# quziyan/NPairLoss

Hardware: NVIDIA H100
Metric: N-pair fwd+bwd samples/sec at B=8192,D=512 (higher is better)
Workload: dtype f32 (3-pass fp16-split wgmma, f32 accumulate)

## Files before the change

### npairloss_b200/csrc/gemm_wgmma.cuh

```cuda
#pragma once
#include <cuda.h>
#include <cuda_runtime.h>
#include <cfloat>
#include <stdint.h>

#include "kernels.cuh"
#include "ptx.cuh"
#include "thresholds.cuh"

namespace npair {

enum { EPI_SIM = 0, EPI_OUT = 1, EPI_SIM_SYM = 2, EPI_SIM_STATS = 3, EPI_SIM_SYM_STATS = 4, EPI_SIM_STORE = 5 };
__host__ __device__ constexpr bool epi_sym(int e) { return e == EPI_SIM_SYM || e == EPI_SIM_SYM_STATS; }
__host__ __device__ constexpr bool epi_stores_s(int e) { return e == EPI_SIM || e == EPI_SIM_SYM || e == EPI_SIM_STORE; }
__host__ __device__ constexpr bool epi_stats(int e) { return e != EPI_OUT && e != EPI_SIM_STORE; }

struct GemmParams {
  int M, Nn;
  int num_kblocks;
  int tiles_m, tiles_n;
  const int2* tile_list;
  int num_tiles_list;
  int splits, kb_per_split;
  float* part;
  float* S;
  long long ldS;
  const float* dev_scale;
  const float* lab_rows;
  const float* lab_cols;
  int self_offset;
  uint32_t* st_minw;
  uint32_t* st_maxw;
  uint32_t* st_maxb;
  uint32_t* st_maxall;
  int* cnt_same;
  int fuse_thr;
  RowArrays ra;
  MiningParams mp;
  BlockScalars* bs;
  float* out;
  long long ldo;
  float alpha, beta;
  int a_row0;
};

template <int NSPLIT, int BK_, int EPI>
struct GemmCfg {
  static constexpr int BM = 128, BN = 256;
  static constexpr int BK = BK_;
  static constexpr int ROW_BYTES = BK * 2;
  static constexpr uint32_t LAYOUT = (ROW_BYTES == 128) ? 1u : 2u;
  static constexpr uint32_t SBO = 8 * ROW_BYTES;
  static constexpr int A_PIECE = BM * ROW_BYTES;
  static constexpr int B_PIECE = BN * ROW_BYTES;
  static constexpr int STAGE_BYTES = NSPLIT * (A_PIECE + B_PIECE);
  static constexpr int NPASS = (NSPLIT == 1) ? 1 : (NSPLIT == 2 ? 3 : 6);
  static constexpr int ACC_STAGE_BYTES = (EPI != EPI_OUT) ? 2 * 64 * 64 * 4 : 0;
  static constexpr int STORE_STAGE_BYTES = (EPI != EPI_OUT) ? 8 * 4096 : 0;
  static constexpr int SMEM_AUX = 2048;
  static constexpr int SMEM_MAX = 227 * 1024;
  static constexpr int STAGES_FIT = (SMEM_MAX - SMEM_AUX - 1024 - ACC_STAGE_BYTES - STORE_STAGE_BYTES) / STAGE_BYTES;
  static constexpr int STAGES = STAGES_FIT > 6 ? 6 : STAGES_FIT;
  static constexpr int SMEM_BYTES = STAGES * STAGE_BYTES + ACC_STAGE_BYTES + STORE_STAGE_BYTES + SMEM_AUX + 1024 ;
  static constexpr int THREADS = 384;
  static_assert(STAGES >= 2 && 16 * STAGES <= 192, "operand ring");
};

__device__ __forceinline__ void pass_pieces(int nsplit, int p, int& sa, int& sb) {
  if (nsplit == 1) { sa = 0; sb = 0; return; }
  if (nsplit == 2) { sa = (p == 2) ? 1 : 0; sb = (p == 1) ? 1 : 0; return; }
  const int A[6] = {0, 0, 1, 1, 0, 2};
  const int B[6] = {0, 1, 0, 1, 2, 0};
  sa = A[p]; sb = B[p];
}

__device__ __forceinline__ void stats32(const float (&v)[32], const float* __restrict__ lab, float lab_i, bool fast, int idx0,
                                        int limit, int self_idx, float& minw, float& maxw, float& maxb, int& cnt) {
  if (fast) {
    float mnw[4] = {FLT_MAX, FLT_MAX, FLT_MAX, FLT_MAX}, mxw[4] = {-FLT_MAX, -FLT_MAX, -FLT_MAX, -FLT_MAX};
    float mxb[4] = {-FLT_MAX, -FLT_MAX, -FLT_MAX, -FLT_MAX};
    int cn[4] = {0, 0, 0, 0};
#pragma unroll
    for (int q = 0; q < 8; ++q) {
      const float4 l4 = *reinterpret_cast<const float4*>(lab + 4 * q);
      const float ll[4] = {l4.x, l4.y, l4.z, l4.w};
#pragma unroll
      for (int e = 0; e < 4; ++e) {
        const float x = v[4 * q + e];
        if (ll[e] == lab_i) { mnw[e] = fminf(mnw[e], x); mxw[e] = fmaxf(mxw[e], x); ++cn[e]; }
        else mxb[e] = fmaxf(mxb[e], x);
      }
    }
    minw = fminf(minw, fminf(fminf(mnw[0], mnw[1]), fminf(mnw[2], mnw[3])));
    maxw = fmaxf(maxw, fmaxf(fmaxf(mxw[0], mxw[1]), fmaxf(mxw[2], mxw[3])));
    maxb = fmaxf(maxb, fmaxf(fmaxf(mxb[0], mxb[1]), fmaxf(mxb[2], mxb[3])));
    cnt += (cn[0] + cn[1]) + (cn[2] + cn[3]);
  } else {
#pragma unroll
    for (int c = 0; c < 32; ++c) {
      const int idx = idx0 + c;
      const bool valid = (idx < limit) && (idx != self_idx);
      const bool same = (lab[c] == lab_i);
      if (valid && same) { minw = fminf(minw, v[c]); maxw = fmaxf(maxw, v[c]); ++cnt; }
      if (valid && !same) maxb = fmaxf(maxb, v[c]);
    }
  }
}

__device__ __forceinline__ float max32(const float (&v)[32]) {
  float m[8];
#pragma unroll
  for (int e = 0; e < 8; ++e) m[e] = fmaxf(fmaxf(v[e], v[8 + e]), fmaxf(v[16 + e], v[24 + e]));
  return fmaxf(fmaxf(fmaxf(m[0], m[1]), fmaxf(m[2], m[3])), fmaxf(fmaxf(m[4], m[5]), fmaxf(m[6], m[7])));
}

template <int NSPLIT, bool BF16, int EPI, int BK_>
__global__ void __launch_bounds__(384, 1)
split_gemm_kernel(const __grid_constant__ CUtensorMap tmapA, const __grid_constant__ CUtensorMap tmapB,
                  const __grid_constant__ CUtensorMap tmapS, const GemmParams p) {
  using Cfg = GemmCfg<NSPLIT, BK_, EPI>;
  const int worker = static_cast<int>(blockIdx.x), num_workers = static_cast<int>(gridDim.x);
  constexpr int BM = Cfg::BM, BN = Cfg::BN, BK = Cfg::BK, STAGES = Cfg::STAGES;
  constexpr bool SYM = epi_sym(EPI), STORE = epi_stores_s(EPI), STATS = epi_stats(EPI);
  extern __shared__ uint8_t smem_raw[];
  uint8_t* smem = smem_raw + ((1024u - (ptx::smem_u32(smem_raw) & 1023u)) & 1023u);
  uint8_t* acc_stage = smem + STAGES * Cfg::STAGE_BYTES;
  uint8_t* store_stage = acc_stage + Cfg::ACC_STAGE_BYTES;
  uint8_t* aux = store_stage + Cfg::STORE_STAGE_BYTES;
  uint64_t* full_bar = reinterpret_cast<uint64_t*>(aux);
  uint64_t* empty_bar = full_bar + STAGES;
  float* s_lab = reinterpret_cast<float*>(aux + 256);
  float* s_labr = reinterpret_cast<float*>(aux + 256 + 1024);
  float2* s_rng = reinterpret_cast<float2*>(aux + 256 + 1024 + 512);

  const int warp = threadIdx.x >> 5, lane = threadIdx.x & 31;
  const int num_tiles = p.tile_list ? p.num_tiles_list : p.tiles_m * p.tiles_n * p.splits;
  const float inv_scale = p.dev_scale ? *p.dev_scale : 1.f;
  const float out_scale = (EPI != EPI_OUT) ? inv_scale * inv_scale : 1.f;
  const float alpha = p.alpha * inv_scale;

  if (warp == 0 && lane == 0) {
    ptx::prefetch_tmap(&tmapA);
    ptx::prefetch_tmap(&tmapB);
    if (STORE) ptx::prefetch_tmap(&tmapS);
  }
  if (warp == 1 && lane == 0) {
    for (int s = 0; s < STAGES; ++s) { ptx::mbar_init(&full_bar[s], 1); ptx::mbar_init(&empty_bar[s], 8); }
    ptx::fence_mbar_init();
  }
  __syncthreads();

  if (warp == 0) {
    if (lane == 0) {
      int stage = 0; uint32_t phase = 0;
      for (int tile = worker; tile < num_tiles; tile += num_workers) {
        const int mn = tile / p.splits, split = tile - mn * p.splits;
        int m_blk = mn / p.tiles_n, n_blk = mn % p.tiles_n;
        if (p.tile_list) { const int2 tl = p.tile_list[tile]; m_blk = tl.x; n_blk = tl.y; }
        const int kb0 = split * p.kb_per_split, kb1 = min(p.num_kblocks, kb0 + p.kb_per_split);
        for (int kb = kb0; kb < kb1; ++kb) {
          ptx::mbar_wait(&empty_bar[stage], phase ^ 1);
          uint8_t* st = smem + stage * Cfg::STAGE_BYTES;
          ptx::mbar_arrive_expect_tx(&full_bar[stage], Cfg::STAGE_BYTES);
#pragma unroll
          for (int s = 0; s < NSPLIT; ++s) {
            ptx::tma_load_3d(st + s * Cfg::A_PIECE, &tmapA, &full_bar[stage], kb * BK, m_blk * BM + (EPI == EPI_SIM_STORE ? p.a_row0 : 0), s);
            ptx::tma_load_3d(st + NSPLIT * Cfg::A_PIECE + s * Cfg::B_PIECE, &tmapB, &full_bar[stage], kb * BK, n_blk * BN, s);
          }
          if (++stage == STAGES) { stage = 0; phase ^= 1; }
        }
      }
    }
  } else if (warp >= 4) {
    const int cw = warp - 4;
    const int g = cw >> 2, wi = warp & 3;
    const int ew = 2 * g + (wi & 1);
    const int half = wi >> 1;
    const int et = threadIdx.x - 128;
    uint8_t* const accs = acc_stage + g * (64 * 256);
    uint8_t* const stg = store_stage + cw * 4096;
    int stage = 0; uint32_t phase = 0;
    for (int tile = worker; tile < num_tiles; tile += num_workers) {
      const int mn = tile / p.splits, split = tile - mn * p.splits;
      int m_blk = mn / p.tiles_n, n_blk = mn % p.tiles_n;
      if (p.tile_list) { const int2 tl = p.tile_list[tile]; m_blk = tl.x; n_blk = tl.y; }
      const int kb0 = split * p.kb_per_split, kb1 = min(p.num_kblocks, kb0 + p.kb_per_split);
      const int row = m_blk * BM + ew * 32 + lane;
      const int col_base = n_blk * BN;
      float lab_i = 0.f;
      if (STATS) {
        asm volatile("bar.sync 1, 256;" ::: "memory");
        s_lab[et] = (col_base + et < p.Nn) ? p.lab_cols[col_base + et] : 0.f;
        if (row < p.M) lab_i = p.lab_rows[row];
        if (SYM && half == 0) s_labr[ew * 32 + lane] = lab_i;
        asm volatile("bar.sync 1, 256;" ::: "memory");
        {
          const float lc = s_lab[cw * 32 + lane];
          float mn = lc, mx = lc;
#pragma unroll
          for (int o = 16; o > 0; o >>= 1) { mn = fminf(mn, __shfl_xor_sync(0xffffffffu, mn, o)); mx = fmaxf(mx, __shfl_xor_sync(0xffffffffu, mx, o)); }
          if (lane == 0) s_rng[cw] = make_float2(mn, mx);
          if (SYM && cw < 4) {
            const float lr = s_labr[cw * 32 + lane];
            float rn = lr, rx = lr;
#pragma unroll
            for (int o = 16; o > 0; o >>= 1) { rn = fminf(rn, __shfl_xor_sync(0xffffffffu, rn, o)); rx = fmaxf(rx, __shfl_xor_sync(0xffffffffu, rx, o)); }
            if (lane == 0) s_rng[8 + cw] = make_float2(rn, rx);
          }
        }
        asm volatile("bar.sync 1, 256;" ::: "memory");
      }

      float acc[128];
#pragma unroll
      for (int i = 0; i < 128; ++i) acc[i] = 0.f;
      for (int kb = kb0; kb < kb1; ++kb) {
        ptx::mbar_wait(&full_bar[stage], phase);
        const uint32_t a0 = ptx::smem_u32(smem + stage * Cfg::STAGE_BYTES) + g * 64 * Cfg::ROW_BYTES;
        const uint32_t b0 = ptx::smem_u32(smem + stage * Cfg::STAGE_BYTES) + NSPLIT * Cfg::A_PIECE;
        ptx::wgmma_fence();
#pragma unroll
        for (int ps = 0; ps < Cfg::NPASS; ++ps) {
          int sa, sb;
          pass_pieces(NSPLIT, ps, sa, sb);
#pragma unroll
          for (int k4 = 0; k4 < BK / 16; ++k4) {
            const uint64_t ad = ptx::make_kmajor_desc(a0 + sa * Cfg::A_PIECE + k4 * 32, Cfg::SBO, Cfg::LAYOUT);
            const uint64_t bd = ptx::make_kmajor_desc(b0 + sb * Cfg::B_PIECE + k4 * 32, Cfg::SBO, Cfg::LAYOUT);
            ptx::wgmma_m64n256k16_ss<BF16>(acc, ad, bd, 1u);
          }
        }
        ptx::wgmma_commit();
        ptx::wgmma_wait<0>();
        ptx::fence_regs(acc);
        __syncwarp();
        if (lane == 0) ptx::mbar_arrive(&empty_bar[stage]);
        if (++stage == STAGES) { stage = 0; phase ^= 1; }
      }

      if (EPI == EPI_OUT) {
        float* obase = p.splits > 1 ? p.part + static_cast<long long>(split) * p.M * p.ldo : p.out;
        const float beta = p.splits > 1 ? 0.f : p.beta;
        const int rbase = m_blk * BM + g * 64 + wi * 16 + (lane >> 2);
#pragma unroll
        for (int j = 0; j < 32; ++j) {
          const int col = col_base + 8 * j + 2 * (lane & 3);
#pragma unroll
          for (int h = 0; h < 2; ++h) {
            const int r = rbase + 8 * h;
            if (r >= p.M || col >= p.Nn) continue;
            float* dst = obase + static_cast<long long>(r) * p.ldo + col;
            float o0 = alpha * acc[4 * j + 2 * h], o1 = alpha * acc[4 * j + 2 * h + 1];
            if (col + 1 < p.Nn && (p.ldo & 1) == 0) {
              if (beta != 0.f) { const float2 old = *reinterpret_cast<const float2*>(dst); o0 += beta * old.x; o1 += beta * old.y; }
              *reinterpret_cast<float2*>(dst) = make_float2(o0, o1);
            } else {
              dst[0] = (beta != 0.f) ? o0 + beta * dst[0] : o0;
              if (col + 1 < p.Nn) dst[1] = (beta != 0.f) ? o1 + beta * dst[1] : o1;
            }
          }
        }
        continue;
      }

      float minw = FLT_MAX, maxw = -FLT_MAX, maxb = -FLT_MAX, maxall = -FLT_MAX;
      int cnt = 0;
      const int self_col = row + p.self_offset;
      const int srow = (wi & 1) * 32 + lane;
#pragma unroll
      for (int cp = 0; cp < 4; ++cp) {
        asm volatile("bar.sync %0, 128;" ::"r"(2 + g) : "memory");
        {
          const int c = lane & 3;
#pragma unroll
          for (int j = 0; j < 8; ++j) {
            const int q = 2 * j + (c >> 1);
#pragma unroll
            for (int h = 0; h < 2; ++h) {
              const int r = wi * 16 + (lane >> 2) + 8 * h;
              *reinterpret_cast<float2*>(accs + r * 256 + ((q ^ (r & 7)) << 4) + (c & 1) * 8) =
                  make_float2(acc[4 * (8 * cp + j) + 2 * h], acc[4 * (8 * cp + j) + 2 * h + 1]);
            }
          }
        }
        asm volatile("bar.sync %0, 128;" ::"r"(2 + g) : "memory");
        const int ch = 2 * cp + half;
        const int col0 = col_base + ch * 32;
        const int cb = col0 >> 7;
        if ((SYM && cb < m_blk) || col0 >= p.Nn) continue;
        float v[32];
        if (STATS) {
#pragma unroll
          for (int q = 0; q < 8; ++q) {
            const float4 t4 = *reinterpret_cast<const float4*>(accs + srow * 256 + (((half * 8 + q) ^ (srow & 7)) << 4));
            v[4 * q] = t4.x * out_scale; v[4 * q + 1] = t4.y * out_scale; v[4 * q + 2] = t4.z * out_scale; v[4 * q + 3] = t4.w * out_scale;
          }
        }
        if (STORE) {
          const int cq = lane & 7;
#pragma unroll
          for (int i = 0; i < 8; ++i) {
            const int rr = 4 * i + (lane >> 3);
            const int grow = m_blk * BM + ew * 32 + rr;
            const int sr = (wi & 1) * 32 + rr;
            float4 o = *reinterpret_cast<const float4*>(accs + sr * 256 + (((half * 8 + cq) ^ (sr & 7)) << 4));
            o.x *= out_scale; o.y *= out_scale; o.z *= out_scale; o.w *= out_scale;
            if (grow < p.M) *reinterpret_cast<float4*>(p.S + static_cast<long long>(grow) * p.ldS + col0 + 4 * cq) = o;
          }
        }
        if (STATS) {
          const float2 rg = s_rng[ch];
          if (__all_sync(0xffffffffu, row >= p.M || lab_i < rg.x || lab_i > rg.y) && col0 + 32 <= p.Nn) {
            if (row < p.M) maxb = fmaxf(maxb, max32(v));
          } else if (row < p.M)
            stats32(v, s_lab + ch * 32, lab_i, col0 + 32 <= p.Nn && (self_col < col0 || self_col >= col0 + 32), col0, p.Nn, self_col,
                    minw, maxw, maxb, cnt);
        }
        if (SYM && cb > m_blk && m_blk * BM + ew * 32 < p.M) {
          if (STORE && lane == 0) ptx::tma_store_wait_read<0>();
          __syncwarp();
#pragma unroll
          for (int c = 0; c < 32; ++c)
            *reinterpret_cast<float*>(stg + c * 128 + ((((lane >> 2) ^ (c & 7))) << 4) + ((lane & 3) << 2)) = v[c];
          if (STORE) ptx::fence_proxy_async_smem();
          __syncwarp();
          if (STORE && lane == 0) { ptx::tma_store_2d(&tmapS, stg, m_blk * BM + ew * 32, col0); ptx::tma_store_commit(); }
          const int gc = col0 + lane;
          float vt[32];
#pragma unroll
          for (int q = 0; q < 8; ++q) {
            const float4 t4 = *reinterpret_cast<const float4*>(stg + lane * 128 + ((q ^ (lane & 7)) << 4));
            vt[4 * q] = t4.x; vt[4 * q + 1] = t4.y; vt[4 * q + 2] = t4.z; vt[4 * q + 3] = t4.w;
          }
          float t_minw = FLT_MAX, t_maxw = -FLT_MAX, t_maxb = -FLT_MAX;
          int t_cnt = 0;
          const int r0 = m_blk * BM + ew * 32;
          const float lab_c = s_lab[ch * 32 + lane];
          const float2 rr = s_rng[8 + ew];
          const bool plain = __all_sync(0xffffffffu, gc >= p.Nn || lab_c < rr.x || lab_c > rr.y) && r0 + 32 <= p.M;
          if (gc < p.Nn) {
            if (plain) t_maxb = max32(vt);
            else stats32(vt, s_labr + ew * 32, lab_c, r0 + 32 <= p.M, r0, p.M, -1, t_minw, t_maxw, t_maxb, t_cnt);
            if (t_cnt) {
              atomicMin(&p.st_minw[gc], f2ord(t_minw));
              atomicMax(&p.st_maxw[gc], f2ord(t_maxw));
              atomicAdd(&p.cnt_same[gc], t_cnt);
            }
            atomicMax(&p.st_maxb[gc], f2ord(t_maxb));
            atomicMax(&p.st_maxall[gc], f2ord(fmaxf(t_maxw, t_maxb)));
          }
        }
      }
      if (STATS && row < p.M) {
        maxall = fmaxf(maxw, maxb);
        if (cnt) {
          atomicMin(&p.st_minw[row], f2ord(minw));
          atomicMax(&p.st_maxw[row], f2ord(maxw));
          atomicAdd(&p.cnt_same[row], cnt);
        }
        atomicMax(&p.st_maxb[row], f2ord(maxb));
        atomicMax(&p.st_maxall[row], f2ord(maxall));
      }
    }
  }
  if (STORE && warp >= 4 && lane == 0) ptx::tma_store_wait<0>();
  __syncthreads();
  if (STATS && p.fuse_thr) {
    volatile int& s_last_cta = *reinterpret_cast<volatile int*>(aux + 192);
    __threadfence();
    __syncthreads();
    if (threadIdx.x == 0) s_last_cta = (atomicAdd(&p.bs->ticket2, 1u) == gridDim.x - 1) ? 1 : 0;
    __syncthreads();
    if (s_last_cta) {
      __threadfence();
      thresholds_one_block(p.ra, p.M, p.Nn, p.mp, p.bs, smem);
      if (threadIdx.x == 0) p.bs->ticket2 = 0;
    }
  }
}

}
```

### npairloss_b200/csrc/grad_fused.cuh

```cuda
#pragma once
#include <cuda.h>
#include <cuda_bf16.h>
#include <cuda_fp16.h>
#include <cuda_runtime.h>
#include <stdint.h>

#include "gemm_wgmma.cuh"
#include "ptx.cuh"

namespace npair {

#define NPAIR_LOG2E_F 1.4426950408889634f

struct FusedGradParams {
  int Q, N, D;
  int num_kblocks;
  int tiles_m, tiles_n;
  int splits, kb_per_split;
  int chunk_kb;
  float* part;
  const float* S;
  const float* rowrec;
  const float* colrec;
  int self_offset;
  float inv_world, log2_world;
  float sgn_p, sgn_n;
  float* out; long long ldo;
  float alpha, beta;
  const float* dev_scale;
  int m_blk0;
};

template <int NSPLIT>
struct FusedCfg {
  static constexpr int BM = 128, BN = 256, BK = 32;
  static constexpr int B_PIECE = BN * 64;
  static constexpr int S_TILE = BM * 128;
  static constexpr int CREC = BK * 32;
  static constexpr int STAGE_BYTES = NSPLIT * B_PIECE + S_TILE + CREC;
  static constexpr int NPASS = (NSPLIT == 1) ? 1 : (NSPLIT == 2 ? 3 : 6);
  static constexpr int STAGES_FIT = (227 * 1024 - 2048) / STAGE_BYTES;
  static constexpr int STAGES = STAGES_FIT > 6 ? 6 : STAGES_FIT;
  static constexpr int SMEM_BYTES = STAGES * STAGE_BYTES + 1024  + 1024 ;
  static constexpr int THREADS = 384;
};

template <int NSPLIT, bool BF16>
__device__ __forceinline__ void split_pair(float a, float b, uint32_t (&out)[3]) {
  if (NSPLIT == 1) {
    out[0] = static_cast<uint32_t>(__bfloat16_as_ushort(__float2bfloat16_rn(a))) | (static_cast<uint32_t>(__bfloat16_as_ushort(__float2bfloat16_rn(b))) << 16);
  } else if (NSPLIT == 2) {
    const __half2 h = __floats2half2_rn(a, b);
    const float2 hf = __half22float2(h);
    const __half2 l = __floats2half2_rn(a - hf.x, b - hf.y);
    out[0] = *reinterpret_cast<const uint32_t*>(&h);
    out[1] = *reinterpret_cast<const uint32_t*>(&l);
  } else {
    const __nv_bfloat162 h = __floats2bfloat162_rn(a, b);
    const float2 hf = __bfloat1622float2(h);
    const float r1a = a - hf.x, r1b = b - hf.y;
    const __nv_bfloat162 m = __floats2bfloat162_rn(r1a, r1b);
    const float2 mf = __bfloat1622float2(m);
    const __nv_bfloat162 l = __floats2bfloat162_rn(r1a - mf.x, r1b - mf.y);
    out[0] = *reinterpret_cast<const uint32_t*>(&h);
    out[1] = *reinterpret_cast<const uint32_t*>(&m);
    out[2] = *reinterpret_cast<const uint32_t*>(&l);
  }
}

__device__ __forceinline__ void red_add_v2(float* dst, float a, float b) {
  asm volatile("red.global.add.v2.f32 [%0], {%1, %2};" ::"l"(dst), "f"(a), "f"(b) : "memory");
}
__device__ __forceinline__ void red_add_f32(float* dst, float a) {
  asm volatile("red.global.add.f32 [%0], %1;" ::"l"(dst), "f"(a) : "memory");
}

__device__ __forceinline__ void bulk_copy_g2s(void* smem_dst, const void* gsrc, uint32_t bytes, uint64_t* bar) {
  asm volatile("cp.async.bulk.shared::cluster.global.mbarrier::complete_tx::bytes [%0], [%1], %2, [%3];"
               ::"r"(ptx::smem_u32(smem_dst)), "l"(reinterpret_cast<uint64_t>(gsrc)), "r"(bytes), "r"(ptx::smem_u32(bar))
               : "memory");
}

__device__ __forceinline__ int chunk_end(int c0, int kb0, int kb1, int ch, int key) {
  if (ch <= 0) return kb1;
  if (c0 == kb0) { const int first = max(1, (((key & 7) + 1) * ch) >> 3); return min(kb1, kb0 + first); }
  return min(kb1, c0 + ch);
}

struct RowRec { float m2r, tn, m2, lab, tp, cA; int self_col; };

__device__ __forceinline__ float pair_weight(float s, const float4* __restrict__ rec, const RowRec& r, int m, const FusedGradParams& p) {
  float g;
  const float4 ca = rec[0];
  if (ca.w != r.lab) {
    const float key = s * p.sgn_n;
    float e1, e2;
    asm("ex2.approx.ftz.f32 %0, %1;" : "=f"(e1) : "f"(key <= r.tn ? fmaf(s, NPAIR_LOG2E_F, -r.m2r) : -INFINITY));
    asm("ex2.approx.ftz.f32 %0, %1;" : "=f"(e2) : "f"(key <= ca.y ? fmaf(s, NPAIR_LOG2E_F, -ca.x) : -INFINITY));
    g = e1 + e2;
  } else {
    const float4 cb = rec[1];
    float e1, e2;
    asm("ex2.approx.ftz.f32 %0, %1;" : "=f"(e1) : "f"(fmaf(s, NPAIR_LOG2E_F, -r.m2)));
    asm("ex2.approx.ftz.f32 %0, %1;" : "=f"(e2) : "f"(fmaf(s, NPAIR_LOG2E_F, -ca.z)));
    const float key = s * p.sgn_p;
    const float w1 = (key <= r.tp) ? e1 * r.cA : 0.f;
    const float w2 = (key <= cb.x) ? e2 * cb.y : 0.f;
    g = fmaf(w2, p.inv_world, w1);
  }
  return (m == r.self_col || m >= p.N) ? 0.f : g;
}

__device__ __forceinline__ RowRec load_rowrec(const FusedGradParams& p, int row) {
  RowRec r;
  r.m2 = 0.f; r.m2r = INFINITY; r.tp = -INFINITY; r.tn = -INFINITY; r.cA = 0.f; r.lab = 0.f;
  r.self_col = row + p.self_offset;
  if (row < p.Q) {
    const float4 a = *reinterpret_cast<const float4*>(p.rowrec + 8ll * row);
    const float4 b = *reinterpret_cast<const float4*>(p.rowrec + 8ll * row + 4);
    r.m2r = a.x - p.log2_world; r.tn = a.y; r.m2 = a.z; r.lab = a.w; r.tp = b.x; r.cA = b.y;
  }
  return r;
}

template <int NSPLIT, bool BF16>
__global__ void __launch_bounds__(384, 1)
fused_grad_kernel(const __grid_constant__ CUtensorMap tmapB, const __grid_constant__ CUtensorMap tmapS, const FusedGradParams p) {
  using Cfg = FusedCfg<NSPLIT>;
  const int worker = static_cast<int>(blockIdx.x), num_workers = static_cast<int>(gridDim.x);
  constexpr int BM = Cfg::BM, BN = Cfg::BN, BK = Cfg::BK, STAGES = Cfg::STAGES;
  extern __shared__ uint8_t smem_raw[];
  uint8_t* smem = smem_raw + ((1024u - (ptx::smem_u32(smem_raw) & 1023u)) & 1023u);
  uint8_t* aux = smem + STAGES * Cfg::STAGE_BYTES;
  uint64_t* full_bar = reinterpret_cast<uint64_t*>(aux);
  uint64_t* empty_bar = full_bar + STAGES;

  const int warp = threadIdx.x >> 5, lane = threadIdx.x & 31;
  const int num_tiles = p.tiles_m * p.tiles_n * p.splits;
  const float inv_scale = p.dev_scale ? *p.dev_scale : 1.f;
  const float alpha = p.alpha * inv_scale;

  if (warp == 8 && lane == 0) {
    ptx::prefetch_tmap(&tmapB); ptx::prefetch_tmap(&tmapS);
    for (int s = 0; s < STAGES; ++s) { ptx::mbar_init(&full_bar[s], 1); ptx::mbar_init(&empty_bar[s], 8); }
    ptx::fence_mbar_init();
  }
  __syncthreads();

  if (warp >= 8) {
    asm volatile("setmaxnreg.dec.sync.aligned.u32 40;");
    if (warp == 8 && lane == 0) {
      int stage = 0; uint32_t phase = 0;
      for (int tile = worker; tile < num_tiles; tile += num_workers) {
        const int mn = tile / p.splits, split = tile - mn * p.splits;
        const int m_blk = mn / p.tiles_n, n_blk = mn % p.tiles_n;
        const int kb0 = split * p.kb_per_split, kb1 = min(p.num_kblocks, kb0 + p.kb_per_split);
        for (int kb = kb0; kb < kb1; ++kb) {
          ptx::mbar_wait(&empty_bar[stage], phase ^ 1);
          const int m0 = kb * BK;
          const uint32_t crec_bytes = static_cast<uint32_t>(min(BK, p.N - m0)) * 32u;
          uint8_t* st = smem + stage * Cfg::STAGE_BYTES;
          ptx::mbar_arrive_expect_tx(&full_bar[stage], NSPLIT * Cfg::B_PIECE + Cfg::S_TILE + crec_bytes);
#pragma unroll
          for (int s = 0; s < NSPLIT; ++s)
            ptx::tma_load_3d(st + s * Cfg::B_PIECE, &tmapB, &full_bar[stage], m0, n_blk * BN, s);
          ptx::tma_load_2d(st + NSPLIT * Cfg::B_PIECE, &tmapS, &full_bar[stage], m0, m_blk * BM);
          bulk_copy_g2s(st + NSPLIT * Cfg::B_PIECE + Cfg::S_TILE, p.colrec + 8ll * m0, crec_bytes, &full_bar[stage]);
          if (++stage == STAGES) { stage = 0; phase ^= 1; }
        }
      }
    }
  } else {
    asm volatile("setmaxnreg.inc.sync.aligned.u32 232;");
    const int g = warp >> 2, wi = warp & 3;
    const int c4 = lane & 3;
    const int rl0 = g * 64 + wi * 16 + (lane >> 2);
    int stage = 0; uint32_t phase = 0;
    for (int tile = worker; tile < num_tiles; tile += num_workers) {
      const int mn = tile / p.splits, split = tile - mn * p.splits;
      const int m_blk = mn / p.tiles_n, n_blk = mn % p.tiles_n;
      const int kb0 = split * p.kb_per_split, kb1 = min(p.num_kblocks, kb0 + p.kb_per_split);
      const int ckey = ((p.m_blk0 + m_blk) >> 1) + n_blk + split;
      float* obase = p.splits > 1 ? p.part + static_cast<long long>(split) * p.Q * p.ldo : p.out;
      const float beta = p.splits > 1 ? 0.f : p.beta;
      float acc[128];
      for (int c0 = kb0, c1; c0 < kb1; c0 = c1) {
        c1 = chunk_end(c0, kb0, kb1, p.chunk_kb, ckey);
        for (int kb = c0; kb < c1; ++kb) {
          ptx::mbar_wait(&full_bar[stage], phase);
          uint8_t* st = smem + stage * Cfg::STAGE_BYTES;
          const uint8_t* s_tile = st + NSPLIT * Cfg::B_PIECE;
          const float4* crec = reinterpret_cast<const float4*>(s_tile + Cfg::S_TILE);
          const uint32_t b0 = ptx::smem_u32(st);
#pragma unroll
          for (int k2 = 0; k2 < BK / 16; ++k2) {
            uint32_t af[NSPLIT][4];
            RowRec rr[2];
#pragma unroll
            for (int h = 0; h < 2; ++h) rr[h] = load_rowrec(p, m_blk * BM + rl0 + 8 * h);
#pragma unroll
            for (int t = 0; t < 2; ++t) {
              const int k = 16 * k2 + 8 * t + 2 * c4;
              const int m = kb * BK + k;
#pragma unroll
              for (int h = 0; h < 2; ++h) {
                const int rl = rl0 + 8 * h;
                const float2 s2 = *reinterpret_cast<const float2*>(s_tile + rl * 128 + (((k >> 2) ^ (rl & 7)) << 4) + (k & 3) * 4);
                const float w0 = pair_weight(s2.x, crec + 2 * k, rr[h], m, p);
                const float w1 = pair_weight(s2.y, crec + 2 * k + 2, rr[h], m + 1, p);
                uint32_t o[3];
                split_pair<NSPLIT, BF16>(w0, w1, o);
#pragma unroll
                for (int s = 0; s < NSPLIT; ++s) af[s][2 * t + h] = o[s];
              }
            }
            ptx::wgmma_fence();
#pragma unroll
            for (int ps = 0; ps < Cfg::NPASS; ++ps) {
              int sa, sb;
              pass_pieces(NSPLIT, ps, sa, sb);
              const uint64_t bd = ptx::make_kmajor_desc(b0 + sb * Cfg::B_PIECE + k2 * 32, 512u, 2u);
              ptx::wgmma_m64n256k16_rs<BF16>(acc, af[sa], bd, ((kb - c0) | ps | k2) != 0 ? 1u : 0u);
            }
            ptx::wgmma_commit();
            ptx::wgmma_wait<0>();
            ptx::fence_regs(acc);
          }
          __syncwarp();
          if (lane == 0) ptx::mbar_arrive(&empty_bar[stage]);
          if (++stage == STAGES) { stage = 0; phase ^= 1; }
        }
        const bool first = (c0 == kb0);
#pragma unroll
        for (int j = 0; j < 32; ++j) {
          const int col = n_blk * BN + 8 * j + 2 * c4;
#pragma unroll
          for (int h = 0; h < 2; ++h) {
            const int row = m_blk * BM + rl0 + 8 * h;
            if (row >= p.Q || col >= p.D) continue;
            float* dst = obase + static_cast<long long>(row) * p.ldo + col;
            float o0 = alpha * acc[4 * j + 2 * h], o1 = alpha * acc[4 * j + 2 * h + 1];
            if (col + 1 < p.D && (p.ldo & 1) == 0) {
              if (first) {
                if (beta != 0.f) { const float2 old = *reinterpret_cast<const float2*>(dst); o0 += beta * old.x; o1 += beta * old.y; }
                *reinterpret_cast<float2*>(dst) = make_float2(o0, o1);
              } else red_add_v2(dst, o0, o1);
            } else {
              if (first) dst[0] = (beta != 0.f) ? o0 + beta * dst[0] : o0; else red_add_f32(dst, o0);
              if (col + 1 < p.D) { if (first) dst[1] = (beta != 0.f) ? o1 + beta * dst[1] : o1; else red_add_f32(dst + 1, o1); }
            }
          }
        }
      }
    }
  }
}

}
```

Baseline: 8.022 million.

## Overlap wgmma with A-fragment build and rebalance registers via setmaxnreg

The similarity GEMM now waits with wgmma_wait<1> and releases the previous smem stage one iteration late, so consecutive K blocks' wgmma groups can overlap. It also adds producer/consumer register reallocation with setmaxnreg. The fused gradient GEMM double-buffers the register A fragments so the pair-weight computation for the next k-step runs while the current wgmma is in flight. It also hoists row records out of the inner loop and rewrites pair_weight branch-free with selects. In exchange, register pressure rises and release ordering becomes more delicate, and the branch-free pair_weight evaluates both label paths every time.

New measurement: 8.875 million, median of 6. 1.11x the previous value.

```diff
diff --git a/npairloss_b200/csrc/gemm_wgmma.cuh b/npairloss_b200/csrc/gemm_wgmma.cuh
--- a/npairloss_b200/csrc/gemm_wgmma.cuh
+++ b/npairloss_b200/csrc/gemm_wgmma.cuh
@@ -150,8 +150,9 @@
   }
   __syncthreads();
 
-  if (warp == 0) {
-    if (lane == 0) {
+  if (warp < 4) {
+    asm volatile("setmaxnreg.dec.sync.aligned.u32 40;");
+    if (warp == 0 && lane == 0) {
       int stage = 0; uint32_t phase = 0;
       for (int tile = worker; tile < num_tiles; tile += num_workers) {
         const int mn = tile / p.splits, split = tile - mn * p.splits;
@@ -171,7 +172,11 @@
         }
       }
     }
-  } else if (warp >= 4) {
+    __syncwarp();
+    asm volatile("bar.sync 4, 384;" ::: "memory");
+    asm volatile("setmaxnreg.inc.sync.aligned.u32 168;");
+  } else {
+    asm volatile("setmaxnreg.inc.sync.aligned.u32 232;");
     const int cw = warp - 4;
     const int g = cw >> 2, wi = warp & 3;
     const int ew = 2 * g + (wi & 1);
@@ -214,6 +219,11 @@
       float acc[128];
 #pragma unroll
       for (int i = 0; i < 128; ++i) acc[i] = 0.f;
+      auto release = [&](int st_idx) {
+        __syncwarp();
+        if (lane == 0) ptx::mbar_arrive(&empty_bar[st_idx]);
+      };
+      int prev = stage;
       for (int kb = kb0; kb < kb1; ++kb) {
         ptx::mbar_wait(&full_bar[stage], phase);
         const uint32_t a0 = ptx::smem_u32(smem + stage * Cfg::STAGE_BYTES) + g * 64 * Cfg::ROW_BYTES;
@@ -231,12 +241,14 @@
           }
         }
         ptx::wgmma_commit();
-        ptx::wgmma_wait<0>();
-        ptx::fence_regs(acc);
-        __syncwarp();
-        if (lane == 0) ptx::mbar_arrive(&empty_bar[stage]);
+        ptx::wgmma_wait<1>();
+        if (kb != kb0) release(prev);
+        prev = stage;
         if (++stage == STAGES) { stage = 0; phase ^= 1; }
       }
+      ptx::wgmma_wait<0>();
+      ptx::fence_regs(acc);
+      if (kb1 > kb0) release(prev);
 
       if (EPI == EPI_OUT) {
         float* obase = p.splits > 1 ? p.part + static_cast<long long>(split) * p.M * p.ldo : p.out;
@@ -362,8 +374,11 @@
         atomicMax(&p.st_maxall[row], f2ord(maxall));
       }
     }
-  }
-  if (STORE && warp >= 4 && lane == 0) ptx::tma_store_wait<0>();
+    if (STORE && lane == 0) ptx::tma_store_wait<0>();
+    __syncwarp();
+    asm volatile("setmaxnreg.dec.sync.aligned.u32 168;");
+    asm volatile("bar.arrive 4, 384;" ::: "memory");
+  }
   __syncthreads();
   if (STATS && p.fuse_thr) {
     volatile int& s_last_cta = *reinterpret_cast<volatile int*>(aux + 192);
diff --git a/npairloss_b200/csrc/grad_fused.cuh b/npairloss_b200/csrc/grad_fused.cuh
--- a/npairloss_b200/csrc/grad_fused.cuh
+++ b/npairloss_b200/csrc/grad_fused.cuh
@@ -89,25 +89,23 @@
 
 struct RowRec { float m2r, tn, m2, lab, tp, cA; int self_col; };
 
-__device__ __forceinline__ float pair_weight(float s, const float4* __restrict__ rec, const RowRec& r, int m, const FusedGradParams& p) {
-  float g;
-  const float4 ca = rec[0];
-  if (ca.w != r.lab) {
-    const float key = s * p.sgn_n;
-    float e1, e2;
-    asm("ex2.approx.ftz.f32 %0, %1;" : "=f"(e1) : "f"(key <= r.tn ? fmaf(s, NPAIR_LOG2E_F, -r.m2r) : -INFINITY));
-    asm("ex2.approx.ftz.f32 %0, %1;" : "=f"(e2) : "f"(key <= ca.y ? fmaf(s, NPAIR_LOG2E_F, -ca.x) : -INFINITY));
-    g = e1 + e2;
-  } else {
-    const float4 cb = rec[1];
-    float e1, e2;
-    asm("ex2.approx.ftz.f32 %0, %1;" : "=f"(e1) : "f"(fmaf(s, NPAIR_LOG2E_F, -r.m2)));
-    asm("ex2.approx.ftz.f32 %0, %1;" : "=f"(e2) : "f"(fmaf(s, NPAIR_LOG2E_F, -ca.z)));
-    const float key = s * p.sgn_p;
-    const float w1 = (key <= r.tp) ? e1 * r.cA : 0.f;
-    const float w2 = (key <= cb.x) ? e2 * cb.y : 0.f;
-    g = fmaf(w2, p.inv_world, w1);
-  }
+__device__ __forceinline__ float select_f32(bool c, float a, float b) {
+  float r;
+  asm("{\n\t.reg .pred q;\n\tsetp.ne.b32 q, %3, 0;\n\tselp.f32 %0, %1, %2, q;\n\t}" : "=f"(r) : "f"(a), "f"(b), "r"(static_cast<int>(c)));
+  return r;
+}
+__device__ __forceinline__ float pair_weight(float s, const float4& ca, const float4& cb, const RowRec& r, int m, const FusedGradParams& p) {
+  const bool same = !(ca.w != r.lab);
+  const float kn = s * p.sgn_n;
+  const float a1 = select_f32(same, fmaf(s, NPAIR_LOG2E_F, -r.m2), select_f32(kn <= r.tn, fmaf(s, NPAIR_LOG2E_F, -r.m2r), -INFINITY));
+  const float a2 = select_f32(same, fmaf(s, NPAIR_LOG2E_F, -ca.z), select_f32(kn <= ca.y, fmaf(s, NPAIR_LOG2E_F, -ca.x), -INFINITY));
+  float e1, e2;
+  asm("ex2.approx.ftz.f32 %0, %1;" : "=f"(e1) : "f"(a1));
+  asm("ex2.approx.ftz.f32 %0, %1;" : "=f"(e2) : "f"(a2));
+  const float kp = s * p.sgn_p;
+  const float w1 = select_f32(kp <= r.tp, e1 * r.cA, 0.f);
+  const float w2 = select_f32(kp <= cb.x, e2 * cb.y, 0.f);
+  const float g = select_f32(same, fmaf(w2, p.inv_world, w1), e1 + e2);
   return (m == r.self_col || m >= p.N) ? 0.f : g;
 }
 
@@ -172,10 +170,37 @@
     }
   } else {
     asm volatile("setmaxnreg.inc.sync.aligned.u32 232;");
+    constexpr int KSTEPS = BK / 16;
+    static_assert(KSTEPS % 2 == 0, "a K block's first step must use A buffer 0");
     const int g = warp >> 2, wi = warp & 3;
     const int c4 = lane & 3;
     const int rl0 = g * 64 + wi * 16 + (lane >> 2);
     int stage = 0; uint32_t phase = 0;
+    auto build = [&](uint32_t (&af)[NSPLIT][4], const RowRec (&rr)[2], int st_idx, int kb, int k2) {
+      const uint8_t* s_tile = smem + st_idx * Cfg::STAGE_BYTES + NSPLIT * Cfg::B_PIECE;
+      const float4* crec = reinterpret_cast<const float4*>(s_tile + Cfg::S_TILE);
+#pragma unroll
+      for (int t = 0; t < 2; ++t) {
+        const int k = 16 * k2 + 8 * t + 2 * c4;
+        const int m = kb * BK + k;
+        const float4 ca0 = crec[2 * k], cb0 = crec[2 * k + 1], ca1 = crec[2 * k + 2], cb1 = crec[2 * k + 3];
+#pragma unroll
+        for (int h = 0; h < 2; ++h) {
+          const int rl = rl0 + 8 * h;
+          const float2 s2 = *reinterpret_cast<const float2*>(s_tile + rl * 128 + (((k >> 2) ^ (rl & 7)) << 4) + (k & 3) * 4);
+          const float w0 = pair_weight(s2.x, ca0, cb0, rr[h], m, p);
+          const float w1 = pair_weight(s2.y, ca1, cb1, rr[h], m + 1, p);
+          uint32_t o[3];
+          split_pair<NSPLIT, BF16>(w0, w1, o);
+#pragma unroll
+          for (int s = 0; s < NSPLIT; ++s) af[s][2 * t + h] = o[s];
+        }
+      }
+    };
+    auto release = [&](int st_idx) {
+      __syncwarp();
+      if (lane == 0) ptx::mbar_arrive(&empty_bar[st_idx]);
+    };
     for (int tile = worker; tile < num_tiles; tile += num_workers) {
       const int mn = tile / p.splits, split = tile - mn * p.splits;
       const int m_blk = mn / p.tiles_n, n_blk = mn % p.tiles_n;
@@ -183,53 +208,45 @@
       const int ckey = ((p.m_blk0 + m_blk) >> 1) + n_blk + split;
       float* obase = p.splits > 1 ? p.part + static_cast<long long>(split) * p.Q * p.ldo : p.out;
       const float beta = p.splits > 1 ? 0.f : p.beta;
+      RowRec rr[2];
+#pragma unroll
+      for (int h = 0; h < 2; ++h) rr[h] = load_rowrec(p, m_blk * BM + rl0 + 8 * h);
       float acc[128];
+      uint32_t af[2][NSPLIT][4];
       for (int c0 = kb0, c1; c0 < kb1; c0 = c1) {
         c1 = chunk_end(c0, kb0, kb1, p.chunk_kb, ckey);
+        ptx::mbar_wait(&full_bar[stage], phase);
+        build(af[0], rr, stage, c0, 0);
+        int prev = stage;
         for (int kb = c0; kb < c1; ++kb) {
-          ptx::mbar_wait(&full_bar[stage], phase);
-          uint8_t* st = smem + stage * Cfg::STAGE_BYTES;
-          const uint8_t* s_tile = st + NSPLIT * Cfg::B_PIECE;
-          const float4* crec = reinterpret_cast<const float4*>(s_tile + Cfg::S_TILE);
-          const uint32_t b0 = ptx::smem_u32(st);
-#pragma unroll
-          for (int k2 = 0; k2 < BK / 16; ++k2) {
-            uint32_t af[NSPLIT][4];
-            RowRec rr[2];
-#pragma unroll
-            for (int h = 0; h < 2; ++h) rr[h] = load_rowrec(p, m_blk * BM + rl0 + 8 * h);
-#pragma unroll
-            for (int t = 0; t < 2; ++t) {
-              const int k = 16 * k2 + 8 * t + 2 * c4;
-              const int m = kb * BK + k;
-#pragma unroll
-              for (int h = 0; h < 2; ++h) {
-                const int rl = rl0 + 8 * h;
-                const float2 s2 = *reinterpret_cast<const float2*>(s_tile + rl * 128 + (((k >> 2) ^ (rl & 7)) << 4) + (k & 3) * 4);
-                const float w0 = pair_weight(s2.x, crec + 2 * k, rr[h], m, p);
-                const float w1 = pair_weight(s2.y, crec + 2 * k + 2, rr[h], m + 1, p);
-                uint32_t o[3];
-                split_pair<NSPLIT, BF16>(w0, w1, o);
-#pragma unroll
-                for (int s = 0; s < NSPLIT; ++s) af[s][2 * t + h] = o[s];
-              }
-            }
+          const int cur = stage;
+          const uint32_t b0 = ptx::smem_u32(smem + cur * Cfg::STAGE_BYTES);
+          if (++stage == STAGES) { stage = 0; phase ^= 1; }
+#pragma unroll
+          for (int k2 = 0; k2 < KSTEPS; ++k2) {
             ptx::wgmma_fence();
 #pragma unroll
             for (int ps = 0; ps < Cfg::NPASS; ++ps) {
               int sa, sb;
               pass_pieces(NSPLIT, ps, sa, sb);
               const uint64_t bd = ptx::make_kmajor_desc(b0 + sb * Cfg::B_PIECE + k2 * 32, 512u, 2u);
-              ptx::wgmma_m64n256k16_rs<BF16>(acc, af[sa], bd, ((kb - c0) | ps | k2) != 0 ? 1u : 0u);
+              ptx::wgmma_m64n256k16_rs<BF16>(acc, af[k2 & 1][sa], bd, ((kb - c0) | ps | k2) != 0 ? 1u : 0u);
             }
             ptx::wgmma_commit();
-            ptx::wgmma_wait<0>();
-            ptx::fence_regs(acc);
+            ptx::wgmma_wait<1>();
+            if (k2 == 0 && kb != c0) release(prev);
+            if (k2 + 1 < KSTEPS) {
+              build(af[(k2 + 1) & 1], rr, cur, kb, k2 + 1);
+            } else if (kb + 1 < c1) {
+              ptx::mbar_wait(&full_bar[stage], phase);
+              build(af[0], rr, stage, kb + 1, 0);
+            }
           }
-          __syncwarp();
-          if (lane == 0) ptx::mbar_arrive(&empty_bar[stage]);
-          if (++stage == STAGES) { stage = 0; phase ^= 1; }
-        }
+          prev = cur;
+        }
+        ptx::wgmma_wait<0>();
+        ptx::fence_regs(acc);
+        release(prev);
         const bool first = (c0 == kb0);
 #pragma unroll
         for (int j = 0; j < 32; ++j) {
```
